# rezashkv/unlearn-ft

Hardware: AMD Instinct MI355X
Metric: bilevel train-step images/sec @512^2 pruned-SD2.1 (higher is better)
Workload: dtype bf16; 1 GPU; BASELINE configs[1] model+batch (MAC-budget-0.55 SD-2.1 student [ratio 0.556, 223.7 GMAC/img] + dense teacher [402.1 GMAC/img], B=8/GPU, 64x64 latents = 512^2 px, losses 1.0 ddpm(min-SNR 5) + 2.0 distill + 0.1 block) under the bilevel cadence of configs[2] (upper concept-suppression step every 10th iteration, second AdamW); global_batch=8, parallelism=dp1, student_params=483766084, weights=random-init, attention_precision=activation dtype, dist_backend=none, rccl_ranks=0, dp_mode=allreduce, teacher_prefetch=True

## Files before the change

unlearn-ft_amd/csrc/abi_util.hip:

```cpp
#include "common.h"

extern "C" int64_t pdmk_gemm_splitk_workspace_bytes(int64_t M, int N, int splitk) {
    if (M <= 0 || N <= 0) return -1;
    return (int64_t)(splitk > 1 ? splitk : 1) * M * N * 4;
}

extern "C" int64_t pdmk_groupnorm_workspace_bytes(int B, int G) {
    if (B <= 0 || G <= 0) return -1;
    return (int64_t)B * G * 64 * 8;
}

extern "C" int64_t pdmk_groupnorm_bwd_part_workspace_bytes(int G, int gs) {
    if (G <= 0 || gs <= 0) return -1;
    return (int64_t)2048 * 2 * G * gs * 4;
}

extern "C" int64_t pdmk_layernorm_bwd_part_workspace_bytes(int M, int C) {
    if (M <= 0 || C <= 0) return -1;
    return ((int64_t)M / 16 + 1) * 2 * C * 4;
}

extern "C" int64_t pdmk_attn_bwd_workspace_bytes(int B, int H, int Nq, int Nk) {
    if (B <= 0 || H <= 0 || Nq <= 0 || Nk <= 0) return -1;
    if (!(Nk <= 128 && Nq >= 512)) return 0;
    return (int64_t)2 * 16 * B * H * Nk * 64 * 4;
}
```

unlearn-ft_amd/csrc/norm.hip:

```cpp
#include "common.h"
#include "vec.h"

namespace {

constexpr int NT = 256;
constexpr int MAXS = 3;

__global__ void reduce_partials_kernel(const float* __restrict__ part, int nblk, int n, float* __restrict__ out0,
                                       float* __restrict__ out1) {
    const int j = blockIdx.x * NT + threadIdx.x;
    if (j >= 2 * n) return;
    const int per = (nblk + gridDim.y - 1) / gridDim.y;
    const int b0 = blockIdx.y * per, b1 = min(nblk, b0 + per);
    float s0 = 0.f, s1 = 0.f, s2 = 0.f, s3 = 0.f;
    int b = b0;
    for (; b + 3 < b1; b += 4) {
        s0 += part[(long)b * 2 * n + j];
        s1 += part[(long)(b + 1) * 2 * n + j];
        s2 += part[(long)(b + 2) * 2 * n + j];
        s3 += part[(long)(b + 3) * 2 * n + j];
    }
    for (; b < b1; ++b) s0 += part[(long)b * 2 * n + j];
    const float s = (s0 + s1) + (s2 + s3);
    if (b1 > b0) unsafeAtomicAdd(j < n ? out0 + j : out1 + (j - n), s);
// ... 334 lines not shown
                pd[sl][u] = Vec<T>::load_raw(dy + ((long)b * HW + rr) * lddy + c * V);
            }
        }
    }
    if (tid < G) {
        sm[tid] = stats[((long)b * G + tid) * 2];
        sr[tid] = stats[((long)b * G + tid) * 2 + 1];
    }
    __syncthreads();
#pragma unroll
    for (int sl = 0; sl < SLOTS; ++sl) {
        const int c = cb + mp.tpr * sl;
        int g = (c * V) / gs, rem = c * V - g * gs;
#pragma unroll
        for (int e = 0; e < V; ++e) {
            const int ch = c * V + e;
            a1[sl][e] = a2[sl][e] = 0.f;
            mean[sl][e] = rstd[sl][e] = 0.f;
            if (c < nchunks && ch < cr) {
                mean[sl][e] = sm[g];
                rstd[sl][e] = sr[g];
            } else {
                gm[sl][e] = bt[sl][e] = 0.f;
            }
            if (++rem == gs) { rem = 0; ++g; }
        }
    }
    if (active) {
        const int step = mp.rif * UNR;
        for (int r = r0 + ro; r < r1; r += step) {
            Raw cx[SLOTS][UNR], cd[SLOTS][UNR];
#pragma unroll
            for (int sl = 0; sl < SLOTS; ++sl) {
                const int c = cb + mp.tpr * sl;
#pragma unroll
                for (int u = 0; u < UNR; ++u) {
                    cx[sl][u] = px[sl][u];
                    cd[sl][u] = pd[sl][u];
                    const int rn = r + step + u * mp.rif;
                    if (c < nchunks && rn < r1) {
                        px[sl][u] = Vec<T>::load_raw(x + ((long)b * HW + rn) * ldx + c * V);
                        pd[sl][u] = Vec<T>::load_raw(dy + ((long)b * HW + rn) * lddy + c * V);
                    }
                }
            }
#pragma unroll
            for (int sl = 0; sl < SLOTS; ++sl) {
                const int c = cb + mp.tpr * sl;
                if (c < nchunks) {
#pragma unroll
                    for (int u = 0; u < UNR; ++u) {
                        const int rr = r + u * mp.rif;
                        if (rr < r1) {
                            float f[V], d[V];
                            Vec<T>::unpack(cx[sl][u], f);
                            Vec<T>::unpack(cd[sl][u], d);
#pragma unroll
                            for (int e = 0; e < V; ++e) {
                                const float xh = (f[e] - mean[sl][e]) * rstd[sl][e];
                                float dz = d[e];
                                if (silu) dz *= silu_grad_f(xh * gm[sl][e] + bt[sl][e]);
                                a1[sl][e] += dz;
                                a2[sl][e] += dz * xh;
                            }
                        }
                    }
                }
            }
        }
    }
    __shared__ float red[2][GN_MAXC / 8 * V];
    if (active) {
#pragma unroll
        for (int sl = 0; sl < SLOTS; ++sl) {
            const int c = cb + mp.tpr * sl;
            if (c < nchunks) {
#pragma unroll
                for (int e = 0; e < V; ++e) {
                    red[0][ro * C + c * V + e] = a1[sl][e];
                    red[1][ro * C + c * V + e] = a2[sl][e];
                }
            }
        }
    }
    __syncthreads();
    float* slab = part + ((long)blockIdx.y * gridDim.x + blockIdx.x) * 2 * cr;
    for (int ch = tid; ch < cr; ch += NT) {
        float t1 = 0.f, t2 = 0.f;
        for (int rr = 0; rr < mp.rif; ++rr) { t1 += red[0][rr * C + ch]; t2 += red[1][rr * C + ch]; }
        slab[ch] = t2;
        slab[cr + ch] = t1;
        const float gmc = gamma[ch];
        red[0][ch] = gmc * t1;
        red[1][ch] = gmc * t2;
    }
    __syncthreads();
    const int g = tid & 63, qt = tid >> 6;
    float ps = 0.f, pq = 0.f;
    if (g < G)
        for (int i = qt; i < gs; i += 4) { ps += red[0][g * gs + i]; pq += red[1][g * gs + i]; }
    __syncthreads();
    red[0][tid] = ps;
    red[1][tid] = pq;
    __syncthreads();
    if (tid < G) {
        float* gs_ = gpart + (((long)b * gridDim.x + blockIdx.x) * G + tid) * 2;
        gs_[0] = (red[0][tid] + red[0][tid + 64]) + (red[0][tid + 128] + red[0][tid + 192]);
        gs_[1] = (red[1][tid] + red[1][tid + 64]) + (red[1][tid + 128] + red[1][tid + 192]);
    }
}

template <typename T, int UNR, int SLOTS>
__global__ __launch_bounds__(NT) void gn_bwd_apply_kernel(const T* __restrict__ x, const T* __restrict__ dy,
                                                          T* __restrict__ dx, const float* __restrict__ gamma,
                                                          const float* __restrict__ beta,
                                                          const float* __restrict__ stats,
                                                          const float* __restrict__ gpart, int nblk, int HW, int C,
                                                          int ldx, int lddy, int lddx, int G, int gs, int silu,
                                                          int accumulate, int rows_per_blk, const T* __restrict__ add,
                                                          int ldadd) {
    constexpr int V = Vec<T>::N;
    typedef typename Vec<T>::raw Raw;
    const int nchunks = C / V;
    const GnMap2 mp = gn_map2(nchunks);
    const int tid = threadIdx.x, cb = tid % mp.tpr, ro = tid / mp.tpr;
    const int b = blockIdx.y;
    const int r0 = blockIdx.x * rows_per_blk, r1 = min(HW, r0 + rows_per_blk);
    const int cr = G * gs;
    __shared__ double scr[2][NT], d0[64], d1[64];
    __shared__ float sm[64], sr[64];
    const bool active = ro < mp.rif;
    const bool vec_gb = ((reinterpret_cast<uintptr_t>(gamma) | reinterpret_cast<uintptr_t>(beta)) & 15) == 0;
    float gm[SLOTS][V], bt[SLOTS][V];
    Raw px[SLOTS][UNR], pd[SLOTS][UNR];
#pragma unroll
    for (int sl = 0; sl < SLOTS; ++sl) {
        const int c = cb + mp.tpr * sl;
        if (active && c < nchunks && c * V + V <= cr && vec_gb) {
#pragma unroll
            for (int e = 0; e < V; e += 4) {
                const float4 g4 = *reinterpret_cast<const float4*>(gamma + c * V + e), b4 = *reinterpret_cast<const float4*>(beta + c * V + e);
                gm[sl][e] = g4.x; gm[sl][e + 1] = g4.y; gm[sl][e + 2] = g4.z; gm[sl][e + 3] = g4.w;
                bt[sl][e] = b4.x; bt[sl][e + 1] = b4.y; bt[sl][e + 2] = b4.z; bt[sl][e + 3] = b4.w;
            }
        } else {
#pragma unroll
            for (int e = 0; e < V; ++e) {
                const int ch = c * V + e;
                const bool ok = active && c < nchunks && ch < cr;
                gm[sl][e] = ok ? gamma[ch] : 0.f;
                bt[sl][e] = ok ? beta[ch] : 0.f;
            }
        }
#pragma unroll
        for (int u = 0; u < UNR; ++u) {
            const int rr = r0 + ro + u * mp.rif;
            if (active && c < nchunks && rr < r1) {
                px[sl][u] = Vec<T>::load_raw(x + ((long)b * HW + rr) * ldx + c * V);
                pd[sl][u] = Vec<T>::load_raw(dy + ((long)b * HW + rr) * lddy + c * V);
            }
        }
    }
    if (tid < G) {
        sm[tid] = stats[((long)b * G + tid) * 2];
        sr[tid] = stats[((long)b * G + tid) * 2 + 1];
    }
    gn_sum_slabs(gpart, b, nblk, G, d0, d1, scr);
    if (!active) return;
    const float invn = 1.0f / ((float)HW * (float)gs);
    float mean[SLOTS][V], rstd[SLOTS][V], c1[SLOTS][V], c2[SLOTS][V];
#pragma unroll
    for (int sl = 0; sl < SLOTS; ++sl) {
        const int c = cb + mp.tpr * sl;
        int g = (c * V) / gs, rem = c * V - g * gs;
#pragma unroll
        for (int e = 0; e < V; ++e) {
            const int ch = c * V + e;
            mean[sl][e] = rstd[sl][e] = c1[sl][e] = c2[sl][e] = 0.f;
            if (c < nchunks && ch < cr) {
                mean[sl][e] = sm[g];
                rstd[sl][e] = sr[g];
                c1[sl][e] = (float)d0[g] * invn;
                c2[sl][e] = (float)d1[g] * invn;
            }
            if (++rem == gs) { rem = 0; ++g; }
        }
    }
    const int step = mp.rif * UNR;
    for (int r = r0 + ro; r < r1; r += step) {
        Raw cx[SLOTS][UNR], cd[SLOTS][UNR];
#pragma unroll
        for (int sl = 0; sl < SLOTS; ++sl) {
            const int c = cb + mp.tpr * sl;
#pragma unroll
            for (int u = 0; u < UNR; ++u) {
                cx[sl][u] = px[sl][u];
                cd[sl][u] = pd[sl][u];
                const int rn = r + step + u * mp.rif;
                if (c < nchunks && rn < r1) {
                    px[sl][u] = Vec<T>::load_raw(x + ((long)b * HW + rn) * ldx + c * V);
                    pd[sl][u] = Vec<T>::load_raw(dy + ((long)b * HW + rn) * lddy + c * V);
                }
            }
        }
#pragma unroll
        for (int sl = 0; sl < SLOTS; ++sl) {
            const int c = cb + mp.tpr * sl;
            if (c < nchunks) {
#pragma unroll
                for (int u = 0; u < UNR; ++u) {
                    const int rr = r + u * mp.rif;
                    if (rr < r1) {
                        float f[V], d[V], o[V], a2[V];
                        Vec<T>::unpack(cx[sl][u], f);
                        Vec<T>::unpack(cd[sl][u], d);
                        if (accumulate) Vec<T>::load(dx + ((long)b * HW + rr) * lddx + c * V, o);
                        if (add) Vec<T>::load(add + ((long)b * HW + rr) * ldadd + c * V, a2);
#pragma unroll
                        for (int e = 0; e < V; ++e) {
                            const float xh = (f[e] - mean[sl][e]) * rstd[sl][e];
                            float dz = d[e];
                            if (silu) dz *= silu_grad_f(xh * gm[sl][e] + bt[sl][e]);
                            float v = rstd[sl][e] * (gm[sl][e] * dz - c1[sl][e] - xh * c2[sl][e]);
                            if (add) v += a2[e];
                            o[e] = accumulate ? o[e] + v : v;
                        }
                        Vec<T>::store(dx + ((long)b * HW + rr) * lddx + c * V, o);
                    }
                }
            }
        }
    }
}

inline int gn_rows_per_blk(int B, int HW, int sweep, int target_blocks, int max_blk) {
    int nb = (target_blocks + B - 1) / B;
    nb = max(1, min(min(nb, max_blk), HW / max(1, sweep)));
    int rpb = (HW + nb - 1) / nb;
    rpb = (rpb + sweep - 1) / sweep * sweep;
    return rpb;
}

template <typename T>
int gn_fwd(const void* x, void* y, const float* gamma, const float* beta, float* stats, double* ws, int B, int HW,
           int C, int ldx, int ldy, int G, int gs, float eps, int silu, hipStream_t st) {
    constexpr int V = Vec<T>::N;
    if (C % V || ldx % V || ldy % V || G > 64 || G * gs > C || C / V > MAXS * NT || C > GN_MAXC / 8 * V) return -1;
    const GnMap2 mp = gn_map2(C / V);
    float* part = reinterpret_cast<float*>(ws);
    const int rpb_s = gn_rows_per_blk(B, HW, mp.rif * 8, 512, GN_MAXBLK);
    dim3 grid_s((HW + rpb_s - 1) / rpb_s, B);
    const int rpb = gn_rows_per_blk(B, HW, mp.rif * 4, 1024, 1 << 20);
    dim3 grid((HW + rpb - 1) / rpb, B);
    const int slots = (C / V + NT - 1) / NT;
#define PDMK_GNF(S)                                                                                                   \
    do {                                                                                                              \
        hipLaunchKernelGGL((gn_stats_kernel<T, 8, S>), grid_s, dim3(NT), 0, st, (const T*)x, part, HW, C, ldx, G, gs, \
                           rpb_s);                                                                                    \
        hipLaunchKernelGGL((gn_apply_kernel<T, 4, S>), grid, dim3(NT), 0, st, (const T*)x, (T*)y, gamma, beta, part,  \
                           (int)grid_s.x, stats, HW, C, ldx, ldy, G, gs, eps, silu, rpb);                             \
    } while (0)
    if (slots == 1) PDMK_GNF(1);
    else if (slots == 2) PDMK_GNF(2);
    else PDMK_GNF(3);
#undef PDMK_GNF
    PDMK_CHECK_LAUNCH();
    return 0;
}

template <typename T>
int gn_bwd(const void* x, const void* dy, void* dx, const float* gamma, const float* beta, const float* stats,
           float* dgamma, float* dbeta, double* ws, float* part, long part_elems, int B, int HW, int C, int ldx,
           int lddy, int lddx, int G, int gs, int silu, int acc, const void* add, int ldadd, hipStream_t st) {
    constexpr int V = Vec<T>::N;
    if (C % V || ldx % V || lddy % V || lddx % V || G > 64 || G * gs > C || C / V > MAXS * NT || C > GN_MAXC / 8 * V) return -1;
    if (add && ((ldadd % V) || ((uintptr_t)add & 15))) return -1;
    const GnMap2 mp = gn_map2(C / V);
    const int rpb_s = gn_rows_per_blk(B, HW, mp.rif * 4, 512, GN_MAXBLK);
    dim3 grid_s((HW + rpb_s - 1) / rpb_s, B);
    const int nblk = grid_s.x * grid_s.y, cr = G * gs;
    if (!part || (long)nblk * 2 * cr > part_elems) return -1;
    float* gpart = reinterpret_cast<float*>(ws);
    const int rpb = gn_rows_per_blk(B, HW, mp.rif * 2, 1024, 1 << 20);
    dim3 grid((HW + rpb - 1) / rpb, B);
    const int slots = (C / V + NT - 1) / NT;
#define PDMK_GNB(S)                                                                                                   \
    do {                                                                                                              \
        hipLaunchKernelGGL((gn_bwd_stats_kernel<T, 4, S>), grid_s, dim3(NT), 0, st, (const T*)x, (const T*)dy, gamma, \
                           beta, stats, part, gpart, HW, C, ldx, lddy, G, gs, silu, rpb_s);                           \
        launch_reduce_partials(part, nblk, cr, dgamma, dbeta, st);                                                    \
        hipLaunchKernelGGL((gn_bwd_apply_kernel<T, 2, S>), grid, dim3(NT), 0, st, (const T*)x, (const T*)dy, (T*)dx,  \
                           gamma, beta, stats, gpart, (int)grid_s.x, HW, C, ldx, lddy, lddx, G, gs, silu, acc, rpb,   \
                           (const T*)add, ldadd);                                                                     \
    } while (0)
    if (slots == 1) PDMK_GNB(1);
    else if (slots == 2) PDMK_GNB(2);
    else PDMK_GNB(3);
#undef PDMK_GNB
    PDMK_CHECK_LAUNCH();
    return 0;
}

constexpr int LN_MAXS = 5;

template <typename T, int SLOTS>
__global__ __launch_bounds__(NT) void ln_fwd_kernel(const T* __restrict__ x, T* __restrict__ y,
                                                    const float* __restrict__ gamma, const float* __restrict__ beta,
                                                    float* __restrict__ stats, int M, int C, int ldx, int ldy,
                                                    float eps, int rows_per_wave) {
    constexpr int V = Vec<T>::N;
    typedef typename Vec<T>::raw Raw;
    const int lane = threadIdx.x & 63, wave = threadIdx.x >> 6;
    const int mbase = (blockIdx.x * 4 + wave) * rows_per_wave, mend = min(M, mbase + rows_per_wave);
    if (mbase >= M) return;
    const int nchunks = C / V;
    const bool vec_gb = ((reinterpret_cast<uintptr_t>(gamma) | reinterpret_cast<uintptr_t>(beta)) & 15) == 0;
    Raw pre[SLOTS];
#pragma unroll
    for (int sl = 0; sl < SLOTS; ++sl) {
        const int c = lane + 64 * sl;
        if (c < nchunks) pre[sl] = Vec<T>::load_raw(x + (long)mbase * ldx + c * V);
    }
    float gm[SLOTS][V], bt[SLOTS][V];
#pragma unroll
    for (int sl = 0; sl < SLOTS; ++sl) {
        const int c = lane + 64 * sl;
        if (c < nchunks && vec_gb) {
#pragma unroll
            for (int e = 0; e < V; e += 4) {
                const float4 g4 = *reinterpret_cast<const float4*>(gamma + c * V + e), b4 = *reinterpret_cast<const float4*>(beta + c * V + e);
                gm[sl][e] = g4.x; gm[sl][e + 1] = g4.y; gm[sl][e + 2] = g4.z; gm[sl][e + 3] = g4.w;
                bt[sl][e] = b4.x; bt[sl][e + 1] = b4.y; bt[sl][e + 2] = b4.z; bt[sl][e + 3] = b4.w;
            }
        } else {
#pragma unroll
            for (int e = 0; e < V; ++e) {
                gm[sl][e] = c < nchunks ? gamma[c * V + e] : 0.f;
                bt[sl][e] = c < nchunks ? beta[c * V + e] : 0.f;
            }
        }
    }
    const float invC = 1.0f / C;
    for (int m = mbase; m < mend; ++m) {
        float f[SLOTS][V];
        float sum = 0.f;
#pragma unroll
        for (int sl = 0; sl < SLOTS; ++sl) {
            const int c = lane + 64 * sl;
            if (c < nchunks) {
                Vec<T>::unpack(pre[sl], f[sl]);
                if (m + 1 < mend) pre[sl] = Vec<T>::load_raw(x + (long)(m + 1) * ldx + c * V);
#pragma unroll
                for (int e = 0; e < V; ++e) sum += f[sl][e];
            }
        }
        const float mean = wave_sum(sum) * invC;
        float sq = 0.f;
#pragma unroll
        for (int sl = 0; sl < SLOTS; ++sl) {
            const int c = lane + 64 * sl;
            if (c < nchunks) {
#pragma unroll
                for (int e = 0; e < V; ++e) { const float d = f[sl][e] - mean; sq += d * d; }
            }
        }
        const float rstd = rsqrtf(wave_sum(sq) * invC + eps);
        if (lane == 0) { stats[2 * (long)m] = mean; stats[2 * (long)m + 1] = rstd; }
#pragma unroll
        for (int sl = 0; sl < SLOTS; ++sl) {
            const int c = lane + 64 * sl;
            if (c < nchunks) {
                float o[V];
#pragma unroll
                for (int e = 0; e < V; ++e) o[e] = (f[sl][e] - mean) * rstd * gm[sl][e] + bt[sl][e];
                Vec<T>::store(y + (long)m * ldy + c * V, o);
            }
        }
    }
}

template <typename T, int SLOTS, int R>
__global__ __launch_bounds__(NT) void ln_bwd_kernel(const T* __restrict__ x, const T* __restrict__ dy,
                                                    T* __restrict__ dx, const float* __restrict__ gamma,
                                                    const float* __restrict__ stats, float* __restrict__ part,
                                                    int M, int C, int ldx, int lddy,
                                                    int lddx, int accumulate, int rows_per_wave,
                                                    const T* __restrict__ add, int ldadd) {
    constexpr int V = Vec<T>::N;
    const int lane = threadIdx.x & 63, wave = threadIdx.x >> 6;
    const int nchunks = C / V;
    float gm[SLOTS][V], ag[SLOTS][V], ab[SLOTS][V];
#pragma unroll
    for (int sl = 0; sl < SLOTS; ++sl) {
        const int c = lane + 64 * sl;
#pragma unroll
        for (int e = 0; e < V; ++e) {
            ag[sl][e] = ab[sl][e] = 0.f;
            gm[sl][e] = (c < nchunks) ? gamma[c * V + e] : 0.f;
        }
    }
    const int mbase = (blockIdx.x * 4 + wave) * rows_per_wave;
    const int mend = min(M, mbase + rows_per_wave);
    const float invC = 1.0f / C;
    typedef typename Vec<T>::raw Raw;
    Raw px[R][SLOTS], pd[R][SLOTS];
    float pm[R], pr[R];
    auto fetch = [&](int m0) {
#pragma unroll
        for (int q = 0; q < R; ++q) {
            const int m = min(m0 + q, mend - 1);
            pm[q] = stats[2 * (long)m];
            pr[q] = stats[2 * (long)m + 1];
#pragma unroll
            for (int sl = 0; sl < SLOTS; ++sl) {
                const int c = lane + 64 * sl;
                if (c < nchunks) {
                    px[q][sl] = Vec<T>::load_raw(x + (long)m * ldx + c * V);
                    pd[q][sl] = Vec<T>::load_raw(dy + (long)m * lddy + c * V);
                }
            }
        }
    };
    if (mbase < mend) fetch(mbase);
    for (int m0 = mbase; m0 < mend; m0 += R) {
        float xh[R][SLOTS][V], d[R][SLOTS][V], mean[R], rstd[R];
#pragma unroll
        for (int q = 0; q < R; ++q) {
            mean[q] = pm[q];
            rstd[q] = pr[q];
#pragma unroll
            for (int sl = 0; sl < SLOTS; ++sl) {
                const int c = lane + 64 * sl;
                if (c < nchunks) {
                    Vec<T>::unpack(px[q][sl], xh[q][sl]);
                    Vec<T>::unpack(pd[q][sl], d[q][sl]);
                } else {
#pragma unroll
                    for (int e = 0; e < V; ++e) xh[q][sl][e] = d[q][sl][e] = 0.f;
                }
            }
        }
        if (m0 + R < mend) fetch(m0 + R);
#pragma unroll
        for (int q = 0; q < R; ++q) {
            const bool live = m0 + q < mend;
            float s1 = 0.f, s2 = 0.f;
#pragma unroll
            for (int sl = 0; sl < SLOTS; ++sl) {
                const int c = lane + 64 * sl;
#pragma unroll
                for (int e = 0; e < V; ++e) {
                    const float h = (c < nchunks) ? (xh[q][sl][e] - mean[q]) * rstd[q] : 0.f;
                    xh[q][sl][e] = h;
                    if (live) { ab[sl][e] += d[q][sl][e]; ag[sl][e] += d[q][sl][e] * h; }
                    const float g = d[q][sl][e] * gm[sl][e];
                    s1 += g;
                    s2 += g * h;
                }
            }
            s1 = wave_sum(s1) * invC;
            s2 = wave_sum(s2) * invC;
            if (live) {
                const int m = m0 + q;
#pragma unroll
                for (int sl = 0; sl < SLOTS; ++sl) {
                    const int c = lane + 64 * sl;
                    if (c < nchunks) {
                        float o[V], a2[V];
                        if (accumulate) Vec<T>::load(dx + (long)m * lddx + c * V, o);
                        if (add) Vec<T>::load(add + (long)m * ldadd + c * V, a2);
#pragma unroll
                        for (int e = 0; e < V; ++e) {
                            float v = rstd[q] * (d[q][sl][e] * gm[sl][e] - s1 - xh[q][sl][e] * s2);
                            if (add) v += a2[e];
                            o[e] = accumulate ? o[e] + v : v;
                        }
                        Vec<T>::store(dx + (long)m * lddx + c * V, o);
                    }
                }
            }
        }
    }
    __shared__ float red[2][3][64 * V];
#pragma unroll
    for (int sl = 0; sl < SLOTS; ++sl) {
        const int c = lane + 64 * sl;
        __syncthreads();
        if (wave > 0) {
#pragma unroll
            for (int e = 0; e < V; ++e) { red[0][wave - 1][lane * V + e] = ag[sl][e]; red[1][wave - 1][lane * V + e] = ab[sl][e]; }
        }
        __syncthreads();
        if (wave == 0 && c < nchunks) {
#pragma unroll
            for (int e = 0; e < V; ++e) {
                const float g2 = ag[sl][e] + red[0][0][lane * V + e] + red[0][1][lane * V + e] + red[0][2][lane * V + e];
                const float b2 = ab[sl][e] + red[1][0][lane * V + e] + red[1][1][lane * V + e] + red[1][2][lane * V + e];
                float* slab = part + (long)blockIdx.x * 2 * C;
                slab[c * V + e] = g2;
                slab[C + c * V + e] = b2;
            }
        }
    }
}

template <typename T>
int ln_fwd(const void* x, void* y, const float* gamma, const float* beta, float* stats, int M, int C, int ldx, int ldy,
           float eps, hipStream_t st) {
    constexpr int V = Vec<T>::N;
    if (C % V || ldx % V || ldy % V || C / V > LN_MAXS * 64) return -1;
    int rpw = M / 8192;
    rpw = rpw < 1 ? 1 : (rpw > 8 ? 8 : rpw);
    const dim3 grid((M + 4 * rpw - 1) / (4 * rpw));
    const int slots = (C / V + 63) / 64;
#define PDMK_LNF(S) hipLaunchKernelGGL((ln_fwd_kernel<T, S>), grid, dim3(NT), 0, st, (const T*)x, (T*)y, gamma, beta, stats, M, \
                                       C, ldx, ldy, eps, rpw)
    if (slots == 1) PDMK_LNF(1);
    else if (slots == 2) PDMK_LNF(2);
    else if (slots == 3) PDMK_LNF(3);
    else PDMK_LNF(5);
#undef PDMK_LNF
    PDMK_CHECK_LAUNCH();
    return 0;
}
static int ln_bwd_rpw(int M) {
    int rpw = (M + 512 * 4 - 1) / (512 * 4);
    return rpw < 8 ? 8 : (rpw > 64 ? 64 : rpw);
}
template <typename T>
int ln_bwd(const void* x, const void* dy, void* dx, const float* gamma, const float* stats, float* dgamma,
           float* dbeta, float* part, long part_elems, int M, int C, int ldx, int lddy, int lddx, int acc,
           const void* add, int ldadd, hipStream_t st) {
    constexpr int V = Vec<T>::N;
    if (C % V || ldx % V || lddy % V || lddx % V || C / V > LN_MAXS * 64 || (add && (ldadd % V))) return -1;
    const int rpw = ln_bwd_rpw(M);
    const int rows_per_blk = 4 * rpw;
    const dim3 grid((M + rows_per_blk - 1) / rows_per_blk);
    if (!part || (long)grid.x * 2 * C > part_elems) return -1;
    const int slots = (C / V + 63) / 64;
#define PDMK_LNB(S, RR) hipLaunchKernelGGL((ln_bwd_kernel<T, S, RR>), grid, dim3(NT), 0, st, (const T*)x, (const T*)dy, \
                                           (T*)dx, gamma, stats, part, M, C, ldx, lddy, lddx, acc, rpw, (const T*)add, ldadd)
    if (slots <= 1) PDMK_LNB(1, 4);
    else if (slots == 2) PDMK_LNB(2, 2);
    else if (slots == 3) PDMK_LNB(3, 2);
    else PDMK_LNB(LN_MAXS, 1);
#undef PDMK_LNB
    launch_reduce_partials(part, grid.x, C, dgamma, dbeta, st);
    PDMK_CHECK_LAUNCH();
    return 0;
}

}

template <typename T>
int gn_apply_colstat(const void* x, void* y, const float* gamma, const float* beta, float* stats, const int64_t* colstat, int cs_ld,
                     int B, int HW, int C, int ldx, int ldy, int G, int gs, float eps, int silu, hipStream_t st) {
    constexpr int V = Vec<T>::N;
    if (C % V || ldx % V || ldy % V || G > 64 || G * gs > C || C / V > MAXS * NT) return -1;
    const GnMap2 mp = gn_map2(C / V);
    const int rpb = gn_rows_per_blk(B, HW, mp.rif * 4, 1024, 1 << 20);
    dim3 grid((HW + rpb - 1) / rpb, B);
    const int slots = (C / V + NT - 1) / NT;
#define PDMK_GNA(S)                                                                                                   \
    hipLaunchKernelGGL((gn_apply_kernel<T, 4, S>), grid, dim3(NT), 0, st, (const T*)x, (T*)y, gamma, beta, reinterpret_cast<const float*>(colstat), -1, stats, \
                       HW, C, ldx, ldy, G, gs, eps, silu, rpb, cs_ld)
    if (slots == 1) PDMK_GNA(1);
    else if (slots == 2) PDMK_GNA(2);
    else PDMK_GNA(3);
#undef PDMK_GNA
    PDMK_CHECK_LAUNCH();
    return 0;
}

extern "C" int pdmk_groupnorm_apply_colstat(const void* x, void* y, const float* gamma, const float* beta, float* stats,
                                            const int64_t* colstat, int cs_ld, int cs_col0, int B, int HW, int C, int ldx, int ldy,
                                            int G, int gs, float eps, int silu, int dtype, pdmk_stream stream) {
    if (!x || !y || !gamma || !beta || !stats || !colstat || B <= 0 || HW <= 0 || C <= 0 || G <= 0 || gs <= 0 || cs_col0 < 0 ||
        cs_ld < cs_col0 + G * gs)
        return -1;
    hipStream_t st = reinterpret_cast<hipStream_t>(stream);
    if (dtype == PDMK_BF16) return gn_apply_colstat<bf16>(x, y, gamma, beta, stats, colstat + cs_col0, cs_ld, B, HW, C, ldx, ldy, G, gs, eps, silu, st);
    if (dtype == PDMK_F32) return gn_apply_colstat<float>(x, y, gamma, beta, stats, colstat + cs_col0, cs_ld, B, HW, C, ldx, ldy, G, gs, eps, silu, st);
    return -2;
}

extern "C" int pdmk_groupnorm_fwd(const void* x, void* y, const float* gamma, const float* beta, float* stats,
                                  double* ws, int B, int HW, int C, int ldx, int ldy, int G, int gs, float eps,
                                  int silu, int dtype, pdmk_stream stream) {
    if (!x || !y || !gamma || !beta || !stats || !ws || B <= 0 || HW <= 0 || G <= 0 || gs <= 0) return -1;
    PDMK_DISPATCH(dtype, gn_fwd, x, y, gamma, beta, stats, ws, B, HW, C, ldx, ldy, G, gs, eps, silu,
                  (hipStream_t)stream);
}
extern "C" int pdmk_groupnorm_bwd(const void* x, const void* dy, void* dx, const float* gamma, const float* beta,
                                  const float* stats, float* dgamma, float* dbeta, double* ws, float* part_ws,
                                  int64_t part_ws_elems, int B, int HW, int C, int ldx, int lddy, int lddx, int G,
                                  int gs, int silu, int accumulate_dx, const void* add, int ldadd, int dtype,
                                  pdmk_stream stream) {
    if (!x || !dy || !dx || !gamma || !beta || !stats || (!dgamma != !dbeta) || !ws || B <= 0 || HW <= 0) return -1;
    PDMK_DISPATCH(dtype, gn_bwd, x, dy, dx, gamma, beta, stats, dgamma, dbeta, ws, part_ws, (long)part_ws_elems, B, HW,
                  C, ldx, lddy, lddx, G, gs, silu, accumulate_dx, add, ldadd, (hipStream_t)stream);
}
extern "C" int pdmk_groupnorm_bwd_partial_dims(int B, int HW, int C, int G, int gs, int dtype, int32_t* nblk, int32_t* n) {
    if (!nblk || !n || B <= 0 || HW <= 0 || C <= 0) return -1;
    const int V = dtype == PDMK_BF16 ? 8 : 4;
    if (C % V) return -1;
    const GnMap2 mp = gn_map2(C / V);
    const int rpb_s = gn_rows_per_blk(B, HW, mp.rif * 4, 512, GN_MAXBLK);
    *nblk = ((HW + rpb_s - 1) / rpb_s) * B;
    *n = G * gs;
    return 0;
}
extern "C" int pdmk_layernorm_bwd_partial_dims(int M, int C, int32_t* nblk, int32_t* n) {
    if (!nblk || !n || M <= 0 || C <= 0) return -1;
    const int rpw = ln_bwd_rpw(M);
    *nblk = (M + 4 * rpw - 1) / (4 * rpw);
    *n = C;
    return 0;
}
extern "C" int pdmk_reduce_partials_group(const pdmk_partial_item* items, int n_items, pdmk_stream stream) {
    if (!items || n_items <= 0 || n_items > PDMK_PARTIAL_GROUP_MAX) return -1;
    PartialGroup gr;
    int nmax = 0;
    for (int i = 0; i < n_items; ++i) {
        if (!items[i].part || !items[i].out0 || !items[i].out1 || items[i].nblk <= 0 || items[i].n <= 0) return -1;
        gr.it[i] = items[i];
        nmax = items[i].n > nmax ? items[i].n : nmax;
    }
    for (int i = n_items; i < PDMK_PARTIAL_GROUP_MAX; ++i) gr.it[i] = items[0];
    hipLaunchKernelGGL(reduce_partials_group_kernel, dim3((2 * nmax + NT - 1) / NT, n_items * 8), dim3(NT), 0,
                       (hipStream_t)stream, gr);
    PDMK_CHECK_LAUNCH();
    return 0;
}
extern "C" int pdmk_layernorm_fwd(const void* x, void* y, const float* gamma, const float* beta, float* stats, int M,
                                  int C, int ldx, int ldy, float eps, int dtype, pdmk_stream stream) {
    if (!x || !y || !gamma || !beta || !stats || M <= 0) return -1;
    PDMK_DISPATCH(dtype, ln_fwd, x, y, gamma, beta, stats, M, C, ldx, ldy, eps, (hipStream_t)stream);
}
extern "C" int pdmk_layernorm_bwd(const void* x, const void* dy, void* dx, const float* gamma, const float* stats,
                                  float* dgamma, float* dbeta, float* part_ws, int64_t part_ws_elems, int M, int C,
                                  int ldx, int lddy, int lddx, int accumulate_dx, const void* add, int ldadd, int dtype,
                                  pdmk_stream stream) {
    if (!x || !dy || !dx || !gamma || !stats || (!dgamma != !dbeta) || M <= 0) return -1;
    PDMK_DISPATCH(dtype, ln_bwd, x, dy, dx, gamma, stats, dgamma, dbeta, part_ws, (long)part_ws_elems, M, C, ldx, lddy,
                  lddx, accumulate_dx, add, ldadd, (hipStream_t)stream);
}
```

Before: 186.2 images/s.

## Pack multiple LayerNorm rows per wave with sub-wave lane groups and LDS gamma

Rewrites the LayerNorm forward and backward kernels so a wave can process several rows at once, using lane groups sized to the channel count (LPR) and shuffle reductions within each group. Gamma and beta are staged in shared memory instead of per-thread registers. The backward kernel folds its per-lane dgamma/dbeta accumulators with a butterfly shuffle before the cross-wave reduction, and picks a new rows-per-block and partial-count heuristic. The goal is higher lane utilisation and lower register pressure when channel counts are small, such as the attention LayerNorms in the SD U-Net. The change adds environment-variable overrides and moves the workspace sizing next to the new block count.

```diff
diff --git a/unlearn-ft_amd/csrc/abi_util.hip b/unlearn-ft_amd/csrc/abi_util.hip
--- a/unlearn-ft_amd/csrc/abi_util.hip
+++ b/unlearn-ft_amd/csrc/abi_util.hip
@@ -15,10 +15,6 @@
     return (int64_t)2048 * 2 * G * gs * 4;
 }
 
-extern "C" int64_t pdmk_layernorm_bwd_part_workspace_bytes(int M, int C) {
-    if (M <= 0 || C <= 0) return -1;
-    return ((int64_t)M / 16 + 1) * 2 * C * 4;
-}
 
 extern "C" int64_t pdmk_attn_bwd_workspace_bytes(int B, int H, int Nq, int Nk) {
     if (B <= 0 || H <= 0 || Nq <= 0 || Nk <= 0) return -1;
diff --git a/unlearn-ft_amd/csrc/norm.hip b/unlearn-ft_amd/csrc/norm.hip
--- a/unlearn-ft_amd/csrc/norm.hip
+++ b/unlearn-ft_amd/csrc/norm.hip
@@ -660,204 +660,248 @@
 }
 
 constexpr int LN_MAXS = 5;
-
-template <typename T, int SLOTS>
-__global__ __launch_bounds__(NT) void ln_fwd_kernel(const T* __restrict__ x, T* __restrict__ y,
+constexpr int LN_NW = NT / 64;
+
+template <int LPR>
+__device__ __forceinline__ float ln_group_sum(float v) {
+#pragma unroll
+    for (int o = LPR / 2; o > 0; o >>= 1) v += __shfl_xor(v, o, 64);
+    return v;
+}
+#define PDMK_LN_CLASS(nchunks, X)               \
+    do {                                        \
+        if ((nchunks) <= 40) X(8, 5, false);    \
+        else if ((nchunks) <= 80) X(16, 5, false);  \
+        else if ((nchunks) <= 128) X(32, 4, true);  \
+        else if ((nchunks) <= 160) X(32, 5, true);  \
+        else if ((nchunks) <= 192) X(64, 3, true);  \
+        else X(64, 5, false);                   \
+    } while (0)
+inline int ln_rows_per_pass(int nchunks) { return nchunks <= 40 ? 8 : (nchunks <= 80 ? 4 : (nchunks <= 160 ? 2 : 1)); }
+
+static int ln_env_int(const char* name, int* cache) {
+    static int dynamic = -1;
+    if (dynamic < 0) dynamic = getenv("PDMK_ENV_DYNAMIC") ? 1 : 0;
+    if (*cache < 0 || dynamic) {
+        const char* e = getenv(name);
+        *cache = e ? max(0, atoi(e)) : 0;
+    }
+    return *cache;
+}
+
+template <typename T, int LPR, int SLOTS>
+__global__ __launch_bounds__(NT, 4) void ln_fwd_kernel(const T* __restrict__ x, T* __restrict__ y,
                                                     const float* __restrict__ gamma, const float* __restrict__ beta,
                                                     float* __restrict__ stats, int M, int C, int ldx, int ldy,
-                                                    float eps, int rows_per_wave) {
-    constexpr int V = Vec<T>::N;
+                                                    float eps, int passes) {
+    constexpr int V = Vec<T>::N, R = 64 / LPR;
     typedef typename Vec<T>::raw Raw;
-    const int lane = threadIdx.x & 63, wave = threadIdx.x >> 6;
-    const int mbase = (blockIdx.x * 4 + wave) * rows_per_wave, mend = min(M, mbase + rows_per_wave);
+    const int lane = threadIdx.x & 63, wave = threadIdx.x >> 6, li = lane % LPR, sub = lane / LPR;
+    const int mbase = (blockIdx.x * LN_NW + wave) * passes * R, mend = min(M, mbase + passes * R);
+    const int nchunks = C / V;
+    constexpr int CW = SLOTS * LPR * V;
+    __shared__ __attribute__((aligned(16))) float sg[CW], sb[CW];
+    float ga[(CW + NT - 1) / NT], ba[(CW + NT - 1) / NT];
+#pragma unroll
+    for (int k = 0; k < (CW + NT - 1) / NT; ++k) {
+        const int i = threadIdx.x + k * NT;
+        ga[k] = i < C ? gamma[i] : 0.f;
+        ba[k] = i < C ? beta[i] : 0.f;
+    }
+    Raw pre[SLOTS];
+    if (mbase < M) {
+        const T* xr = x + (long)min(mbase + sub, mend - 1) * ldx + li * V;
+#pragma unroll
+        for (int sl = 0; sl < SLOTS; ++sl)
+            if (li + LPR * sl < nchunks) pre[sl] = Vec<T>::load_raw(xr + sl * LPR * V);
+    }
+#pragma unroll
+    for (int k = 0; k < (CW + NT - 1) / NT; ++k) {
+        const int i = threadIdx.x + k * NT;
+        if (i < CW) { sg[i] = ga[k]; sb[i] = ba[k]; }
+    }
+    __syncthreads();
     if (mbase >= M) return;
-    const int nchunks = C / V;
-    const bool vec_gb = ((reinterpret_cast<uintptr_t>(gamma) | reinterpret_cast<uintptr_t>(beta)) & 15) == 0;
-    Raw pre[SLOTS];
-#pragma unroll
-    for (int sl = 0; sl < SLOTS; ++sl) {
-        const int c = lane + 64 * sl;
-        if (c < nchunks) pre[sl] = Vec<T>::load_raw(x + (long)mbase * ldx + c * V);
-    }
-    float gm[SLOTS][V], bt[SLOTS][V];
-#pragma unroll
-    for (int sl = 0; sl < SLOTS; ++sl) {
-        const int c = lane + 64 * sl;
-        if (c < nchunks && vec_gb) {
-#pragma unroll
-            for (int e = 0; e < V; e += 4) {
-                const float4 g4 = *reinterpret_cast<const float4*>(gamma + c * V + e), b4 = *reinterpret_cast<const float4*>(beta + c * V + e);
-                gm[sl][e] = g4.x; gm[sl][e + 1] = g4.y; gm[sl][e + 2] = g4.z; gm[sl][e + 3] = g4.w;
-                bt[sl][e] = b4.x; bt[sl][e + 1] = b4.y; bt[sl][e + 2] = b4.z; bt[sl][e + 3] = b4.w;
-            }
-        } else {
-#pragma unroll
-            for (int e = 0; e < V; ++e) {
-                gm[sl][e] = c < nchunks ? gamma[c * V + e] : 0.f;
-                bt[sl][e] = c < nchunks ? beta[c * V + e] : 0.f;
-            }
-        }
-    }
     const float invC = 1.0f / C;
-    for (int m = mbase; m < mend; ++m) {
+    for (int m0 = mbase; m0 < mend; m0 += R) {
+        const int m = m0 + sub;
+        const bool live = m < mend;
+        const T* xn = x + (long)min(m + R, mend - 1) * ldx + li * V;
+        T* yr = y + (long)m * ldy + li * V;
         float f[SLOTS][V];
         float sum = 0.f;
 #pragma unroll
         for (int sl = 0; sl < SLOTS; ++sl) {
-            const int c = lane + 64 * sl;
+            const int c = li + LPR * sl;
             if (c < nchunks) {
                 Vec<T>::unpack(pre[sl], f[sl]);
-                if (m + 1 < mend) pre[sl] = Vec<T>::load_raw(x + (long)(m + 1) * ldx + c * V);
+                if (m0 + R < mend) pre[sl] = Vec<T>::load_raw(xn + sl * LPR * V);
 #pragma unroll
                 for (int e = 0; e < V; ++e) sum += f[sl][e];
             }
         }
-        const float mean = wave_sum(sum) * invC;
+        const float mean = ln_group_sum<LPR>(sum) * invC;
         float sq = 0.f;
 #pragma unroll
         for (int sl = 0; sl < SLOTS; ++sl) {
-            const int c = lane + 64 * sl;
+            const int c = li + LPR * sl;
             if (c < nchunks) {
 #pragma unroll
                 for (int e = 0; e < V; ++e) { const float d = f[sl][e] - mean; sq += d * d; }
             }
         }
-        const float rstd = rsqrtf(wave_sum(sq) * invC + eps);
-        if (lane == 0) { stats[2 * (long)m] = mean; stats[2 * (long)m + 1] = rstd; }
+        const float rstd = rsqrtf(ln_group_sum<LPR>(sq) * invC + eps);
+        asm volatile("" ::: "memory");
+        if (live) {
+            if (li == 0) { stats[2 * (long)m] = mean; stats[2 * (long)m + 1] = rstd; }
+#pragma unroll
+            for (int sl = 0; sl < SLOTS; ++sl) {
+                const int c = li + LPR * sl;
+                if (c < nchunks) {
+                    float o[V], gm[V], bt[V];
+#pragma unroll
+                    for (int e = 0; e < V; e += 4) {
+                        Vec<float>::load(sg + c * V + e, gm + e);
+                        Vec<float>::load(sb + c * V + e, bt + e);
+                    }
+#pragma unroll
+                    for (int e = 0; e < V; ++e) o[e] = (f[sl][e] - mean) * rstd * gm[e] + bt[e];
+                    Vec<T>::store(yr + sl * LPR * V, o);
+                }
+            }
+        }
+    }
+}
+
+template <typename T, int LPR, int SLOTS, bool PF>
+__global__ __launch_bounds__(NT, (PF && sizeof(T) == 2 && SLOTS == LN_MAXS) ? 1 : 2)
+void ln_bwd_kernel(const T* __restrict__ x, const T* __restrict__ dy,
+                                                       T* __restrict__ dx, const float* __restrict__ gamma,
+                                                       const float* __restrict__ stats, float* __restrict__ part,
+                                                       int M, int C, int ldx, int lddy,
+                                                       int lddx, int accumulate, int rows_per_blk,
+                                                       const T* __restrict__ add, int ldadd) {
+    constexpr int V = Vec<T>::N, R = 64 / LPR, NACC = 2 * SLOTS * V, NE = NACC / R;
+    static_assert(NACC % R == 0, "the fold halves the sums log2(R) times");
+    typedef typename Vec<T>::raw Raw;
+    const int lane = threadIdx.x & 63, wave = threadIdx.x >> 6, li = lane % LPR, sub = lane / LPR;
+    const int nchunks = C / V;
+    float acc[NACC];
+    constexpr int CW = SLOTS * LPR * V, LDSF = (LN_NW - 1) * NACC * LPR > CW ? (LN_NW - 1) * NACC * LPR : CW;
+    __shared__ __attribute__((aligned(16))) float lds[LDSF];
+    for (int i = threadIdx.x; i < CW; i += NT) lds[i] = i < C ? gamma[i] : 0.f;
+    __syncthreads();
+#pragma unroll
+    for (int i = 0; i < NACC; ++i) acc[i] = 0.f;
+    const int r0 = blockIdx.x * rows_per_blk, r1 = min(M, r0 + rows_per_blk);
+    const float invC = 1.0f / C;
+    Raw px[SLOTS], pd[SLOTS];
+    float pm = 0.f, pr = 0.f;
+#pragma unroll
+    for (int sl = 0; sl < SLOTS; ++sl) px[sl] = pd[sl] = Raw{};
+    auto fetch = [&](int m0) {
+        const int m = min(m0 + sub, r1 - 1);
+        pm = stats[2 * (long)m];
+        pr = stats[2 * (long)m + 1];
+        const T* xr = x + (long)m * ldx + li * V;
+        const T* dr = dy + (long)m * lddy + li * V;
 #pragma unroll
         for (int sl = 0; sl < SLOTS; ++sl) {
-            const int c = lane + 64 * sl;
-            if (c < nchunks) {
-                float o[V];
-#pragma unroll
-                for (int e = 0; e < V; ++e) o[e] = (f[sl][e] - mean) * rstd * gm[sl][e] + bt[sl][e];
-                Vec<T>::store(y + (long)m * ldy + c * V, o);
-            }
-        }
-    }
-}
-
-template <typename T, int SLOTS, int R>
-__global__ __launch_bounds__(NT) void ln_bwd_kernel(const T* __restrict__ x, const T* __restrict__ dy,
-                                                    T* __restrict__ dx, const float* __restrict__ gamma,
-                                                    const float* __restrict__ stats, float* __restrict__ part,
-                                                    int M, int C, int ldx, int lddy,
-                                                    int lddx, int accumulate, int rows_per_wave,
-                                                    const T* __restrict__ add, int ldadd) {
-    constexpr int V = Vec<T>::N;
-    const int lane = threadIdx.x & 63, wave = threadIdx.x >> 6;
-    const int nchunks = C / V;
-    float gm[SLOTS][V], ag[SLOTS][V], ab[SLOTS][V];
-#pragma unroll
-    for (int sl = 0; sl < SLOTS; ++sl) {
-        const int c = lane + 64 * sl;
-#pragma unroll
-        for (int e = 0; e < V; ++e) {
-            ag[sl][e] = ab[sl][e] = 0.f;
-            gm[sl][e] = (c < nchunks) ? gamma[c * V + e] : 0.f;
-        }
-    }
-    const int mbase = (blockIdx.x * 4 + wave) * rows_per_wave;
-    const int mend = min(M, mbase + rows_per_wave);
-    const float invC = 1.0f / C;
-    typedef typename Vec<T>::raw Raw;
-    Raw px[R][SLOTS], pd[R][SLOTS];
-    float pm[R], pr[R];
-    auto fetch = [&](int m0) {
-#pragma unroll
-        for (int q = 0; q < R; ++q) {
-            const int m = min(m0 + q, mend - 1);
-            pm[q] = stats[2 * (long)m];
-            pr[q] = stats[2 * (long)m + 1];
+            if (li + LPR * sl < nchunks) {
+                px[sl] = Vec<T>::load_raw(xr + sl * LPR * V);
+                pd[sl] = Vec<T>::load_raw(dr + sl * LPR * V);
+            }
+        }
+    };
+    int m0 = r0 + wave * R;
+    if (PF && m0 < r1) fetch(m0);
+#pragma unroll 1
+    for (; m0 < r1; m0 += LN_NW * R) {
+        if (!PF) fetch(m0);
+        Raw cx[SLOTS], cd[SLOTS];
+#pragma unroll
+        for (int sl = 0; sl < SLOTS; ++sl) { cx[sl] = px[sl]; cd[sl] = pd[sl]; }
+        const float mean = pm, rstd = pr;
+        if (PF && m0 + LN_NW * R < r1) fetch(m0 + LN_NW * R);
+        const int m = m0 + sub;
+        const bool live = m < r1;
+        const float lv = live ? 1.f : 0.f;
+        float s1 = 0.f, s2 = 0.f;
+        asm volatile("" ::: "memory");
+#pragma unroll
+        for (int sl = 0; sl < SLOTS; ++sl) {
+            float f[V], d[V], gm[V];
+            Vec<T>::unpack(cx[sl], f);
+            Vec<T>::unpack(cd[sl], d);
+            Vec<float>::load(lds + (li + LPR * sl) * V, gm);
+            if (V == 8) Vec<float>::load(lds + (li + LPR * sl) * V + 4, gm + 4);
+#pragma unroll
+            for (int e = 0; e < V; ++e) {
+                const float h = (f[e] - mean) * rstd, dl = d[e] * lv;
+                acc[sl * V + e] += dl * h;
+                acc[(SLOTS + sl) * V + e] += dl;
+                const float g = d[e] * gm[e];
+                s1 += g;
+                s2 += g * h;
+            }
+        }
+        s1 = ln_group_sum<LPR>(s1) * invC;
+        s2 = ln_group_sum<LPR>(s2) * invC;
+        asm volatile("" ::: "memory");
+        if (live) {
+            T* or_ = dx + (long)m * lddx + li * V;
+            const T* ar = add + (long)m * ldadd + li * V;
 #pragma unroll
             for (int sl = 0; sl < SLOTS; ++sl) {
-                const int c = lane + 64 * sl;
+                const int c = li + LPR * sl;
                 if (c < nchunks) {
-                    px[q][sl] = Vec<T>::load_raw(x + (long)m * ldx + c * V);
-                    pd[q][sl] = Vec<T>::load_raw(dy + (long)m * lddy + c * V);
+                    float f[V], d[V], o[V], a2[V], gm[V];
+                    Vec<T>::unpack(cx[sl], f);
+                    Vec<T>::unpack(cd[sl], d);
+                    Vec<float>::load(lds + c * V, gm);
+                    if (V == 8) Vec<float>::load(lds + c * V + 4, gm + 4);
+                    if (accumulate) Vec<T>::load(or_ + sl * LPR * V, o);
+                    if (add) Vec<T>::load(ar + sl * LPR * V, a2);
+#pragma unroll
+                    for (int e = 0; e < V; ++e) {
+                        const float h = (f[e] - mean) * rstd;
+                        float v = rstd * (d[e] * gm[e] - s1 - h * s2);
+                        if (add) v += a2[e];
+                        o[e] = accumulate ? o[e] + v : v;
+                    }
+                    Vec<T>::store(or_ + sl * LPR * V, o);
                 }
             }
         }
-    };
-    if (mbase < mend) fetch(mbase);
-    for (int m0 = mbase; m0 < mend; m0 += R) {
-        float xh[R][SLOTS][V], d[R][SLOTS][V], mean[R], rstd[R];
-#pragma unroll
-        for (int q = 0; q < R; ++q) {
-            mean[q] = pm[q];
-            rstd[q] = pr[q];
-#pragma unroll
-            for (int sl = 0; sl < SLOTS; ++sl) {
-                const int c = lane + 64 * sl;
-                if (c < nchunks) {
-                    Vec<T>::unpack(px[q][sl], xh[q][sl]);
-                    Vec<T>::unpack(pd[q][sl], d[q][sl]);
-                } else {
-#pragma unroll
-                    for (int e = 0; e < V; ++e) xh[q][sl][e] = d[q][sl][e] = 0.f;
-                }
-            }
-        }
-        if (m0 + R < mend) fetch(m0 + R);
-#pragma unroll
-        for (int q = 0; q < R; ++q) {
-            const bool live = m0 + q < mend;
-            float s1 = 0.f, s2 = 0.f;
-#pragma unroll
-            for (int sl = 0; sl < SLOTS; ++sl) {
-                const int c = lane + 64 * sl;
-#pragma unroll
-                for (int e = 0; e < V; ++e) {
-                    const float h = (c < nchunks) ? (xh[q][sl][e] - mean[q]) * rstd[q] : 0.f;
-                    xh[q][sl][e] = h;
-                    if (live) { ab[sl][e] += d[q][sl][e]; ag[sl][e] += d[q][sl][e] * h; }
-                    const float g = d[q][sl][e] * gm[sl][e];
-                    s1 += g;
-                    s2 += g * h;
-                }
-            }
-            s1 = wave_sum(s1) * invC;
-            s2 = wave_sum(s2) * invC;
-            if (live) {
-                const int m = m0 + q;
-#pragma unroll
-                for (int sl = 0; sl < SLOTS; ++sl) {
-                    const int c = lane + 64 * sl;
-                    if (c < nchunks) {
-                        float o[V], a2[V];
-                        if (accumulate) Vec<T>::load(dx + (long)m * lddx + c * V, o);
-                        if (add) Vec<T>::load(add + (long)m * ldadd + c * V, a2);
-#pragma unroll
-                        for (int e = 0; e < V; ++e) {
-                            float v = rstd[q] * (d[q][sl][e] * gm[sl][e] - s1 - xh[q][sl][e] * s2);
-                            if (add) v += a2[e];
-                            o[e] = accumulate ? o[e] + v : v;
-                        }
-                        Vec<T>::store(dx + (long)m * lddx + c * V, o);
-                    }
-                }
-            }
-        }
-    }
-    __shared__ float red[2][3][64 * V];
-#pragma unroll
-    for (int sl = 0; sl < SLOTS; ++sl) {
-        const int c = lane + 64 * sl;
-        __syncthreads();
-        if (wave > 0) {
-#pragma unroll
-            for (int e = 0; e < V; ++e) { red[0][wave - 1][lane * V + e] = ag[sl][e]; red[1][wave - 1][lane * V + e] = ab[sl][e]; }
-        }
-        __syncthreads();
-        if (wave == 0 && c < nchunks) {
-#pragma unroll
-            for (int e = 0; e < V; ++e) {
-                const float g2 = ag[sl][e] + red[0][0][lane * V + e] + red[0][1][lane * V + e] + red[0][2][lane * V + e];
-                const float b2 = ab[sl][e] + red[1][0][lane * V + e] + red[1][1][lane * V + e] + red[1][2][lane * V + e];
-                float* slab = part + (long)blockIdx.x * 2 * C;
-                slab[c * V + e] = g2;
-                slab[C + c * V + e] = b2;
-            }
+    }
+    int off = 0;
+#pragma unroll
+    for (int k = 0; (LPR << k) < 64; ++k) {
+        const int n = NACC >> (k + 1);
+        const bool up = (sub >> k) & 1;
+#pragma unroll
+        for (int i = 0; i < n; ++i) {
+            const float keep = up ? acc[i + n] : acc[i], send = up ? acc[i] : acc[i + n];
+            acc[i] = keep + __shfl_xor(send, LPR << k, 64);
+        }
+        off += up ? n : 0;
+    }
+    float (*red)[NACC * LPR] = reinterpret_cast<float (*)[NACC * LPR]>(lds);
+    __syncthreads();
+    if (wave > 0) {
+#pragma unroll
+        for (int j = 0; j < NE; ++j) red[wave - 1][(off + j) * LPR + li] = acc[j];
+    }
+    __syncthreads();
+    if (wave == 0) {
+        float* slab = part + (long)blockIdx.x * 2 * C;
+#pragma unroll
+        for (int j = 0; j < NE; ++j) {
+            const int idx = off + j, arr = idx / (SLOTS * V), rem = idx - arr * (SLOTS * V), c = li + LPR * (rem / V);
+            float t = acc[j];
+#pragma unroll
+            for (int w = 0; w < LN_NW - 1; ++w) t += red[w][idx * LPR + li];
+            if (c < nchunks) slab[arr * C + c * V + rem % V] = t;
         }
     }
 }
@@ -867,23 +911,30 @@
            float eps, hipStream_t st) {
     constexpr int V = Vec<T>::N;
     if (C % V || ldx % V || ldy % V || C / V > LN_MAXS * 64) return -1;
-    int rpw = M / 8192;
-    rpw = rpw < 1 ? 1 : (rpw > 8 ? 8 : rpw);
-    const dim3 grid((M + 4 * rpw - 1) / (4 * rpw));
-    const int slots = (C / V + 63) / 64;
-#define PDMK_LNF(S) hipLaunchKernelGGL((ln_fwd_kernel<T, S>), grid, dim3(NT), 0, st, (const T*)x, (T*)y, gamma, beta, stats, M, \
-                                       C, ldx, ldy, eps, rpw)
-    if (slots == 1) PDMK_LNF(1);
-    else if (slots == 2) PDMK_LNF(2);
-    else if (slots == 3) PDMK_LNF(3);
-    else PDMK_LNF(5);
+    const int nchunks = C / V, R = ln_rows_per_pass(nchunks);
+    static int forced = -1;
+    int passes = ln_env_int("PDMK_LN_FWD_PASSES", &forced);
+    if (!passes) passes = max(1, min(8, M / (R * LN_NW * 1024)));
+    const int rows_per_blk = LN_NW * R * passes;
+    const dim3 grid((M + rows_per_blk - 1) / rows_per_blk);
+#define PDMK_LNF(L, S, PFB) hipLaunchKernelGGL((ln_fwd_kernel<T, L, S>), grid, dim3(NT), 0, st, (const T*)x, (T*)y, gamma, beta, stats, \
+                                          M, C, ldx, ldy, eps, passes)
+    PDMK_LN_CLASS(nchunks, PDMK_LNF);
 #undef PDMK_LNF
     PDMK_CHECK_LAUNCH();
     return 0;
 }
-static int ln_bwd_rpw(int M) {
-    int rpw = (M + 512 * 4 - 1) / (512 * 4);
-    return rpw < 8 ? 8 : (rpw > 64 ? 64 : rpw);
+static int ln_bwd_rows_per_blk(int M) {
+    static int forced = -1;
+    const int f = ln_env_int("PDMK_LN_BWD_ROWS", &forced);
+    if (f) return f;
+    const int blocks = M > 16384 ? 512 : 256;
+    const int rows = ((M + blocks - 1) / blocks + 7) / 8 * 8;
+    return rows > 128 ? 128 : rows;
+}
+static int ln_bwd_nblk(int M) {
+    const int rpb = ln_bwd_rows_per_blk(M);
+    return (M + rpb - 1) / rpb;
 }
 template <typename T>
 int ln_bwd(const void* x, const void* dy, void* dx, const float* gamma, const float* stats, float* dgamma,
@@ -891,17 +942,13 @@
            const void* add, int ldadd, hipStream_t st) {
     constexpr int V = Vec<T>::N;
     if (C % V || ldx % V || lddy % V || lddx % V || C / V > LN_MAXS * 64 || (add && (ldadd % V))) return -1;
-    const int rpw = ln_bwd_rpw(M);
-    const int rows_per_blk = 4 * rpw;
-    const dim3 grid((M + rows_per_blk - 1) / rows_per_blk);
+    const int rows_per_blk = ln_bwd_rows_per_blk(M);
+    const dim3 grid(ln_bwd_nblk(M));
     if (!part || (long)grid.x * 2 * C > part_elems) return -1;
-    const int slots = (C / V + 63) / 64;
-#define PDMK_LNB(S, RR) hipLaunchKernelGGL((ln_bwd_kernel<T, S, RR>), grid, dim3(NT), 0, st, (const T*)x, (const T*)dy, \
-                                           (T*)dx, gamma, stats, part, M, C, ldx, lddy, lddx, acc, rpw, (const T*)add, ldadd)
-    if (slots <= 1) PDMK_LNB(1, 4);
-    else if (slots == 2) PDMK_LNB(2, 2);
-    else if (slots == 3) PDMK_LNB(3, 2);
-    else PDMK_LNB(LN_MAXS, 1);
+    const int nchunks = C / V;
+#define PDMK_LNB(L, S, PFB) hipLaunchKernelGGL((ln_bwd_kernel<T, L, S, (V == 4 || PFB)>), grid, dim3(NT), 0, st, (const T*)x, (const T*)dy, \
+                                               (T*)dx, gamma, stats, part, M, C, ldx, lddy, lddx, acc, rows_per_blk, (const T*)add, ldadd)
+    PDMK_LN_CLASS(nchunks, PDMK_LNB);
 #undef PDMK_LNB
     launch_reduce_partials(part, grid.x, C, dgamma, dbeta, st);
     PDMK_CHECK_LAUNCH();
@@ -970,10 +1017,15 @@
 }
 extern "C" int pdmk_layernorm_bwd_partial_dims(int M, int C, int32_t* nblk, int32_t* n) {
     if (!nblk || !n || M <= 0 || C <= 0) return -1;
-    const int rpw = ln_bwd_rpw(M);
-    *nblk = (M + 4 * rpw - 1) / (4 * rpw);
+    *nblk = ln_bwd_nblk(M);
     *n = C;
     return 0;
+}
+extern "C" int64_t pdmk_layernorm_bwd_part_workspace_bytes(int M, int C) {
+    if (M <= 0 || C <= 0) return -1;
+    const int64_t rows16 = (int64_t)M / 16 + 1;
+    const int64_t nblk = ln_bwd_nblk(M);
+    return (nblk > rows16 ? nblk : rows16) * 2 * C * 4;
 }
 extern "C" int pdmk_reduce_partials_group(const pdmk_partial_item* items, int n_items, pdmk_stream stream) {
     if (!items || n_items <= 0 || n_items > PDMK_PARTIAL_GROUP_MAX) return -1;
```

After: 188.0 images/s, median of 6. No clear change (+1.0%).
